# zengxianyu/sketchedit

Measured on NVIDIA H100. Metric: images/sec 256x256 CelebA-HQ generator fwd, higher is better.
Workload: dtype bf16

## Files before the change

sketchedit_b200/csrc/se_conv_c8.cu:

```cuda
#include "se_conv_c8.h"

#include <stdlib.h>

#include <atomic>
#include <map>
#include <mutex>
#include <vector>

#include "../../include/sketchedit_b200.h"
#include "se_tc_device.cuh"

namespace se {

constexpr int C8_TH = 16, C8_TW = 8;
constexpr int C8_CONSUMER_WARPS = 8;
__host__ __device__ constexpr int c8_threads(int teams) { return 32 * C8_CONSUMER_WARPS * teams + 32; }
constexpr int C8_MAX_STAGES = 8;

__device__ __forceinline__ void ring_of(int i, int n, int shift, int& slot, uint32_t& phase) {
  if (shift >= 0) { slot = i & (n - 1); phase = (uint32_t)(i >> shift) & 1u; }
  else { const int qd = i / n; slot = i - qd * n; phase = (uint32_t)qd & 1u; }
}

template <int NT, bool kF16, int R64, int M64, int R32, int TEAMS>
// ... 608 lines not shown
  }
  p.step_x = grid % p.tiles_x;
  p.step_y = (grid / p.tiles_x) % p.tiles_y;
  p.step_img = grid / (p.tiles_x * p.tiles_y);
  p.cstep_x = (teams * grid) % p.tiles_x;
  p.cstep_y = (teams * grid / p.tiles_x) % p.tiles_y;
  p.cstep_img = teams * grid / (p.tiles_x * p.tiles_y);
  cudaLaunchConfig_t cfg;
  cudaLaunchAttribute attr;
  c8_launch_config(&cfg, &attr, grid, teams, smem_bytes, p.cluster, stream);
  SE_CUDA_OK(cudaLaunchKernelEx(&cfg, kernel, tmA, p));
  if (c8_log_on()) c8_log_append(p, c, (int)(inst - kC8Insts), teams, grid, total_tiles);
  return 0;
}

}

extern "C" {

int se_c8_log_enable(int on) {
  std::lock_guard<std::mutex> lk(se::g_c8_log_mu);
  se::g_c8_log = on != 0;
  se::g_c8_log_recs.clear();
  se::g_c8_log_label.clear();
  return 0;
}

int se_c8_log_count(void) {
  std::lock_guard<std::mutex> lk(se::g_c8_log_mu);
  return (int)se::g_c8_log_recs.size();
// ... 28 lines not shown
```

sketchedit_b200/csrc/se_conv_c8.h:

```cpp
#pragma once
#include "se_common.cuh"
#include "se_conv_tc.h"

namespace se {

enum { C8_HALO = 0, C8_PERTAP = 1 };
constexpr int C8_MAX_ABUFS = 8;
constexpr int C8_MAX_UNITS = 128;

struct C8Layer {
  TcWeights w;
  int mode = C8_HALO;
  bool resident = false;
  bool stem = false;
  int cb_in = 0;
  int mmas64 = 4;
  int HR = 0, WR = 0;
  int pad_y0 = 0, pad_x0 = 0;
  int a_bytes = 0, a_tx_bytes = 0;
  int8_t tap_cb[MAX_TAPS] = {0};
  int chunks_per_tap = 1;
};

constexpr int C8_MAX_CLS = 4;
// ... 25 lines not shown
  const float* bias;
  EpiParams e;
  int f16;
  int8_t tap_cb[MAX_TAPS];
  int cpt;
  int ncls, cls_bytes;
  int cls_ooy[C8_MAX_CLS], cls_oox[C8_MAX_CLS];
  int cluster;
};

int c8_configure(C8Layer* L, int ntaps, const int8_t* dy, const int8_t* dx, int Ci, int Cout, bool stem, const int8_t* tap_cb = nullptr);
int c8_launch(const ConvParams& c, const C8Layer& L, cudaStream_t stream, const C8Group* grp = nullptr);
int c8_instantiated(const C8Layer& L, bool f16, const std::string& name);
int c8_configure_group(C8Group* G, int ncls, int ntaps, const int8_t (*dy)[8], const int8_t (*dx)[8], const int* ooy, const int* oox, int Ci, int Cout);

bool c8_log_on();
void c8_log_label(const std::string& name);

}
```

sketchedit_b200/csrc/se_engine.cu:

```cuda
#include <stdlib.h>

#include <cuda_fp16.h>

#include <algorithm>
#include <atomic>
#include <cmath>
#include <cstring>
#include <functional>
#include <map>
#include <mutex>
#include <string>
#include <type_traits>
#include <vector>

#include "../../include/sketchedit_b200.h"
#include "se_common.cuh"
#include "se_conv_direct.h"
#include "se_conv_c8.h"
#include "se_cam.h"
#include "se_gemm_split.h"
#include "se_conv_tc.h"
#include "se_misc.h"
#include "se_detail.h"

// ... 552 lines not shown
  } else {
    elems = (size_t)c.B * v.ld * (layout == 2 ? (size_t)(v.H / 2) * (v.W / 2) : (size_t)v.H * v.W) * 8;
  }
  t.bytes = elems * (dtype == 0 ? 4 : 2);
  SE_CUDA_OK(cudaMalloc(&t.p, t.bytes));
  c.m->taps.push_back(t);
  SE_CUDA_OK(cudaMemcpyAsync(t.p, v.p, t.bytes, cudaMemcpyDeviceToDevice, c.stream));
  return 0;
}
#define TAP(...)                  \
  do {                            \
    int _rt = tap(c, __VA_ARGS__); \
    if (_rt) return _rt;          \
  } while (0)

static int run_layer(Ctx& c, Layer& L, const View& in, void* out, int ldo, int choff, int out_c8 = 0) {
  SE_REQUIRE(in.c8 == wants_c8(c, L), "activation layout mismatch at layer " + L.name);
  TAP("in:" + std::string(1, L.net) + "." + L.name, in, L.is_stem ? 3 : in.c8);
  const Spec& s = L.spec;
  const int Ho = s.deconv ? in.H : (in.H + s.stride - 1) / s.stride;
  const int Wo = s.deconv ? in.W : (in.W + s.stride - 1) / s.stride;
  const bool fused = c.prec == SE_PREC_BF16_TC && !L.groups.empty() && in.c8 == 1;
  const bool split = c.split();
  const int n_launch = fused ? (int)L.groups.size() : (int)L.cls.size();
  if (c8_log_on() && !c.dry) c8_log_label(std::string(1, L.net) + "." + L.name);
  for (int li = 0; li < n_launch; ++li) {
    const C8Group* grp = fused ? &L.groups[li] : nullptr;
    ClassW& cw = L.cls[fused ? li * grp->ncls : li];
    ConvParams cp;
    memset(&cp, 0, sizeof(cp));
    cp.x = in.p; cp.in_dt = c.act_dt();
    cp.N = c.B; cp.Hi = in.H; cp.Wi = in.W; cp.Ci = L.Ci; cp.ldx = in.ld;
    if (L.is_stem && !in.c8) {
      cp.ldx = 8;
      cp.Wi = stem_wp(in.W) - 7;
      cp.x_row_pitch = (long long)stem_wp(in.W) * 8;
      cp.x_img_pitch = (long long)in.H * cp.x_row_pitch;
    }
    if (in.c8) {
      cp.in_c8 = 1; cp.x_cb_off = in.cb_off; cp.ldx = in.ld;
// ... 23 lines not shown
    cp.epi = s.act == 1 ? EPI_GATE_RELU : EPI_GATE_ELU;
    cp.scale = split ? 1.0f / (kSplitActScale * cw.s_wscale) : 1.0f;
    cp.colscale = nullptr;
    if (L.fused_pair) {
      SE_REQUIRE(out_c8 == 2 && ldo == 24, "a fused stem pair writes two space-to-depth tensors");
      cp.out_blk_split = 3; cp.out_par_stride = 3; cp.out_blk_jump = 9 * (cp.Hout / 2) * (cp.Wout / 2);
    }
    if (g_timing && !c.dry) {
      const double gc = grp ? grp->ncls : 1.0;
      const double pos = (double)c.B * Ho * Wo * gc, ncls = (double)L.cls.size() / gc;
      const double cin_alg = L.fused_pair ? L.pair_cin_sum / 2.0 : (double)s.cin;
      const double f_alg = 2.0 * pos * s.cout * cin_alg * (s.deconv ? 9.0 : (double)s.k * s.k);
      const double f_exec = 2.0 * pos * s.cout * cin_alg * (s.deconv ? 4.0 : (double)s.k * s.k) * (split ? 3.0 : 1.0);
      const double bytes = ((double)c.B * in.H * in.W * (L.fused_pair ? 8.0 : (double)s.cin) / ncls + pos * (s.cout / 2) + (double)s.cout * s.cin * s.k * s.k / ncls) * c.esz();
      char buf[160];
      snprintf(buf, sizeof(buf), "%s|%s %d->%d k%d s%d d%d @%dx%d", c.tc() ? (split ? "conv_c8_kernel (split-half fp16 x3)" : "conv_c8_kernel") : "conv_direct_kernel",
               s.deconv ? (grp ? (grp->ncls == 4 ? "deconv (4 classes fused)" : "deconv (2 classes fused)") : "deconv-class") : (L.fused_pair ? "stem pair" : "conv"), s.cin, s.cout, s.k, s.stride, s.rate, Ho * cw.osy, Wo * cw.osx);
      c.tag(buf, c.tc() ? 1 : 0, f_alg, f_exec, bytes);
    }
    if (split) CK(c8_launch(cp, cw.c8s, c.stream));
    else if (c.tc()) CK(c8_launch(cp, cw.c8, c.stream, grp));
    else {
      cp.w = cw.w_direct;
      CK(direct_launch(cp, cw.CoutP, c.stream));
    }
  }
  return 0;
}

static void out_dims(const Spec& s, int H, int W, int* Ho, int* Wo) {
  if (s.deconv) { *Ho = 2 * H; *Wo = 2 * W; }
  else { *Ho = (H + s.stride - 1) / s.stride; *Wo = (W + s.stride - 1) / s.stride; }
}

struct Dst { void* p = nullptr; int ld = 0, choff = 0, c8 = -1; };
// ... 32 lines not shown
  return 0;
}

static std::vector<std::string> with_prefix(const std::string& pfx, std::initializer_list<const char*> l, int skip = 0) {
  std::vector<std::string> v;
  for (auto s = l.begin() + skip; s != l.end(); ++s) v.push_back(pfx + *s);
  return v;
}

static int run_head(Ctx& c, char net, const std::string& name, const View& in, int mode, HeadIO io) {
  Layer* L = find_ready(c.m, net, name);
  SE_REQUIRE(L != nullptr && L->is_head, "head layer " + name + ": " + last_error());
  TAP("in:" + std::string(1, net) + "." + name, in, in.c8);
  {
    const double px = (double)c.B * in.H * in.W;
    const int outs = !!io.mask + !!io.mask_bin + !!io.stage + !!io.composed;
    const double bytes = px * ((in.c8 ? 16 : 12) * c.esz() + (io.img ? 12 : 0) + (io.blend ? 4 : 0) + outs * 4 * L->spec.cout + (io.packed ? 8 * c.esz() : 0));
    const double fl = 2.0 * px * 9 * 12 * L->spec.cout;
    c.tag(std::string("head_kernel|12->") + std::to_string(L->spec.cout) + " k3 + " +
              (mode == HEAD_MASK ? "sigmoid+threshold" : mode == HEAD_TANH ? "tanh" : mode == HEAD_COARSE ? "tanh+blend+pack8" : "tanh+soft blend"),
          0, fl, fl, bytes);
  }
  SE_REQUIRE(in.c8 == (c.tc() ? 1 : 0) && in.ld == (c.tc() ? 2 * c.sp() : 12), "head input: dense 12 channels in the mode's storage");
  io.x = in.p; io.B = c.B; io.H = in.H; io.W = in.W; io.mode = mode;
  io.Wp = stem_wp(in.W); io.padl = STEM_PADL; io.no_mask_coarse = c.m->opt[SE_OPT_NO_MASK_COARSE];
  CK(head(io, c.act_dt(), L->w_head_host.data(), L->b_host.data(), L->spec.cout, c.stream));
  return 0;
}

static int run_cam_tc(Ctx& c, const View& f, const float* mask_s, void* out, float* attn_out) {
  SE_REQUIRE(f.c8 == 2 && f.C == 96, "tensor-core attention reads a 96-channel space-to-depth channel-blocked map");
  CamPlan pl;
  int rc = cam_plan(c.B, f.H, f.W, c.attn_limit, attn_out != nullptr, &pl);
  if (rc) return rc;
  Buf fn = c.get(pl.fn_bytes), cs = c.get(pl.cs_bytes), P = c.get(pl.p_bytes);
  if (g_timing && !c.dry) {
    const double L = (double)pl.hs * pl.ws;
    const double fl = 4.0 * c.B * L * L * 96 * 16;
    c.tag("cam_s_kernel + cam_pv_kernel (+ norm, colscale)|contextual attention", 1, fl, 1.5 * fl,
          (double)c.B * f.H * f.W * 96 * 2 * 2 + 2.0 * (double)c.B * pl.KB * pl.hs * pl.ws * 16);
  }
// ... 152 lines not shown
  float* mask_bin = nullptr;
  unsigned char* mask_u8 = nullptr;
  float* x_stage1 = nullptr;
};

static int run_netM(Ctx& c, int H, int W, const NetMIO& io) {
  SE_REQUIRE(io.mask || io.x_stage1, "netM with neither output");
  Act in8, x9;
  int rc = do_pack8(c, &in8, io.x, io.guide, nullptr, H, W, PACK_IMG_ONE, 1.0f, 0);
  if (rc) return rc;
  std::vector<std::string> trunk = with_prefix("", kEncoder);
  trunk.pop_back();
  rc = run_chain(c, 'M', trunk, in8, &x9);
  if (rc) return rc;
  if (io.x_stage1) {
    Act v16;
    rc = run_chain(c, 'M', with_prefix("conv", kDecoder), x9.borrow(), &v16);
    if (rc) return rc;
    HeadIO h{};
    h.stage = io.x_stage1;
    rc = run_head(c, 'M', "conv17", v16.v, HEAD_TANH, h);
    if (rc) return rc;
    c.put(v16);
  }
  if (!io.mask) {
    c.put(x9);
    return 0;
  }
  Act v;
  rc = run_chain(c, 'M', with_prefix("", {"conv10_atrous", "conv_mask_11", "conv_mask_12", "conv_mask_13_upsample_conv", "conv_mask_14",
                                          "conv_mask_15_upsample_conv", "conv_mask_16"}),
                 x9, &v);
  if (rc) return rc;
  Buf scratch;
  HeadIO h{};
  h.mask = io.mask; h.mask_bs = io.mask_bs; h.mask_bin = io.mask_bin; h.mask_u8 = io.mask_u8;
  if (!h.mask_bin) { scratch = c.get((size_t)c.B * H * W * 4); h.mask_bin = (float*)scratch.p; }
  rc = run_head(c, 'M', "conv_mask_17", v.v, HEAD_MASK, h);
  if (rc) return rc;
  c.put(scratch);
  c.put(v);
  return 0;
}

static int run_stem_pair(Ctx& c, Layer& pair, Act in, Buf* st) {
  *st = c.get((size_t)c.B * 24 * (in.v.H / 2) * (in.v.W / 2) * 16);
  int rc = run_layer(c, pair, in.v, st->p, 24, 0, 2);
  if (rc) return rc;
  c.put(in);
  return 0;
}

struct NetGIO {
  const float *x, *x2, *mask, *mask2, *guide;
  float *x_stage1 = nullptr, *x_stage2 = nullptr, *composed = nullptr;
  long long composed_bs = 0;
// ... 27 lines not shown
  Act in;
  if (!pair1) rc = do_pack8(c, &in, io.x, io.guide, io.mask, H, W, PACK_IMG_ONE_MINUS_M, 1.0f, 1);
  if (rc) return rc;
  rc = run_chain(c, 'G', with_prefix("", kEncoder, pair1 ? 1 : 0), pair1 ? Act{pair_half(st1, 0)} : in, nullptr, Dst{cat1.p, cat_ld, 0});
  if (rc) return rc;
  if (!pair1) rc = do_pack8(c, &in, io.x2, io.guide, io.mask2, H, W, style_img, opt[SE_OPT_JOINT_TRAIN_INP] ? 0.0f : 1.0f, 1);
  if (rc) return rc;
  Act style;
  rc = run_chain(c, 'G', with_prefix("w", kEncoder, pair1 ? 1 : 0), pair1 ? Act{pair_half(st1, 1)} : in, &style);
  if (rc) return rc;
  c.put(st1);
  rc = do_pool_broadcast(c, style.v, opt[SE_OPT_POOL_AVG] ? RED_AVG : RED_MAX, cat1.p, cat_ld);
  if (rc) return rc;
  c.put(style);
  Buf xnow = c.get((size_t)c.B * H * stem_wp(W) * 8 * e);
  Act dec;
  rc = run_chain(c, 'G', with_prefix("conv", kDecoder), Act{c.dense(cat1.p, h, w, 192, tc), cat1}, &dec);
  if (rc) return rc;
  c.tag("memset|pad pixels of the packed stage-2 input", 0, 0, 0, (double)xnow.bytes);
  CK(fill_zero(xnow.p, xnow.bytes, c.stream));
  HeadIO coarse{};
  coarse.img = io.x; coarse.blend = io.mask; coarse.stage = io.x_stage1; coarse.packed = xnow.p;
  rc = run_head(c, 'G', "conv17", dec.v, HEAD_COARSE, coarse);
  if (rc) return rc;
  c.put(dec);

  Buf cat2 = c.get((size_t)c.B * h * w * 192 * e);
  Act in2{stem_view(c, xnow.p, H, W), xnow};
  Buf st2;
  if (pair2) {
    rc = run_stem_pair(c, *pair2, in2, &st2);
    if (rc) return rc;
  }
  rc = run_chain(c, 'G', with_prefix("x", kEncoder, pair2 ? 1 : 0), pair2 ? Act{pair_half(st2, 0)} : in2.borrow(), nullptr, Dst{cat2.p, cat_ld, 0});
  if (rc) return rc;
  const int pm_c8 = opt[SE_OPT_USE_CAM] ? (c.split() ? 1 : (tc ? 2 : 0)) : -1;
  Act pm;
  rc = run_chain(c, 'G', with_prefix("pm", {"conv1", "conv2_downsample", "conv3", "conv4_downsample", "conv5", "conv6"}, pair2 ? 1 : 0),
                 pair2 ? Act{pair_half(st2, 1), st2} : in2, &pm, Dst{nullptr, 0, 0, pm_c8});
  if (rc) return rc;
// ... 12 lines not shown
      rc = run_cam_split(c, (const float*)f32.p, h, w, 96, (const float*)ms.p, (float*)o32.p, io.attn);
      if (rc) return rc;
      TAP("out:G.cam.f32", nhwc(o32.p, h, w, 96, 96), 0, 0);
      CK(f32_to_act((const float*)o32.p, 1, camo.p, DT_F16X2, pml, c.B, 96, c.stream));
      c.put(o32); c.put(f32);
    } else {
      rc = tc ? run_cam_tc(c, pm.v, (const float*)ms.p, camo.p, io.attn) : run_cam(c, pm.v, (const float*)ms.p, camo.p, 96, io.attn, 0);
      if (rc) return rc;
    }
    c.put(ms);
    c.put(pm);
    pm = Act{c.dense(camo.p, h, w, 96, tc), camo};
  }
  rc = run_chain(c, 'G', with_prefix("pm", {"conv9", "conv10"}), pm, nullptr, Dst{cat2.p, cat_ld, 96});
  if (rc) return rc;
  rc = run_chain(c, 'G', with_prefix("allconv", kDecoder), Act{c.dense(cat2.p, h, w, 192, tc), cat2}, &dec);
  if (rc) return rc;
  HeadIO fine{};
  fine.stage = io.x_stage2;
  const bool blend = io.composed || io.composed_u8;
  if (blend) {
    fine.img = io.x; fine.blend = io.mask_soft; fine.blend_bs = io.msoft_bs;
    fine.composed = io.composed; fine.composed_bs = io.composed_bs; fine.bgr_u8 = io.composed_u8;
  }
  rc = run_head(c, 'G', "allconv17", dec.v, blend ? HEAD_FINE : HEAD_TANH, fine);
  if (rc) return rc;
  c.put(dec);
  return 0;
}

struct Request {
  const float *image = nullptr, *sketch = nullptr;
  const unsigned char *image_u8 = nullptr, *sketch_u8 = nullptr;
  const float* edit_mask = nullptr;
  const unsigned char* edit_mask_u8 = nullptr;
  float *composed = nullptr, *mask = nullptr;
  long long composed_bs = 0, mask_bs = 0;
  unsigned char *bgr_u8 = nullptr, *mask_u8 = nullptr;
  float *coarse = nullptr, *fine = nullptr, *mask_image = nullptr;
  const float* mask_bin_in = nullptr;
  float* mask_bin_out = nullptr;
  float* attn = nullptr;
// ... 610 lines not shown
```

sketchedit_b200/csrc/se_misc.cu:

```cuda
#include <type_traits>

#include "se_common.cuh"
#include "se_misc.h"

namespace se {

static inline int cdiv(long long a, long long b) { return (int)((a + b - 1) / b); }

struct F32 {
  static constexpr int kHalves = 1;
  static constexpr bool kBlocked = false;
  template <int N = 8>
  __device__ static void load8(const void* x, size_t o, size_t, float (&v)[8]) {
#pragma unroll
    for (int k = 0; k < N; ++k) v[k] = __ldg(static_cast<const float*>(x) + o + k);
  }
  __device__ static void store8(void* y, size_t o, size_t, const float (&v)[8]) {
#pragma unroll
    for (int k = 0; k < 8; ++k) static_cast<float*>(y)[o + k] = v[k];
  }
  __device__ static float get(const void* x, size_t o, size_t) { return __ldg(static_cast<const float*>(x) + o); }
  __device__ static void put(void* y, size_t o, size_t, float v) { static_cast<float*>(y)[o] = v; }
};

// ... 107 lines not shown
      for (int c = 0; c < 3; ++c) v[5 + c] = img[(b * 3 + c) * HW + pix] * a2;
    }
  }
  St::store8(out, o, lo, v);
}

int pack8(const float* img, const float* sketch, const float* mask, void* out, int dt, int B, int H, int W, int Wp, int padl,
          int img_mode, float sketch_scale, int write_mask, cudaStream_t s, int img2_mode) {
  const long long n = (long long)B * H * Wp;
  return with_storage(dt, [&](auto st) {
    pack8_kernel<decltype(st)><<<cdiv(n, 256), 256, 0, s>>>(img, sketch, mask, out, B, H, W, Wp, padl, img_mode, sketch_scale, write_mask,
                                                            img2_mode);
  });
}

template <int COUT>
struct HeadWeights {
  float2 w[9][6][COUT];
  float b[COUT];
};
template <class St, int COUT>
__global__ void __launch_bounds__(128) head_kernel(const __grid_constant__ HeadWeights<COUT> hw, const __grid_constant__ HeadIO io) {
  constexpr bool kPairs = std::is_same<St, Bf16>::value;
  const int H = io.H, W = io.W;
  const long long i = blockIdx.x * (long long)blockDim.x + threadIdx.x;
  const long long HW = (long long)H * W;
  if (i >= io.B * HW) return;
  const long long b = i / HW, pix = i % HW;
  const int yy = (int)(pix / W), xx = (int)(pix % W);
  float2 acc[COUT];
#pragma unroll
  for (int o = 0; o < COUT; ++o) acc[o] = make_float2(kPairs ? 0.0f : hw.b[o], 0.0f);
#pragma unroll
  for (int t = 0; t < 9; ++t) {
    const int iy = yy + t / 3 - 1, ix = xx + t % 3 - 1;
    if (iy < 0 || iy >= H || ix < 0 || ix >= W) continue;
    const long long q = (long long)iy * W + ix;
    float v[2][8];
    if constexpr (St::kBlocked) {
      const size_t o = ((size_t)b * 2 * St::kHalves * HW + q) * 8, blk = (size_t)HW * 8;
      St::load8(io.x, o, 2 * blk, v[0]);
      St::load8(io.x, o + blk, 2 * blk, v[1]);
    } else {
      St::load8(io.x, (size_t)(b * HW + q) * 12, 0, v[0]);
      St::template load8<4>(io.x, (size_t)(b * HW + q) * 12 + 8, 0, v[1]);
    }
#pragma unroll
    for (int p = 0; p < 6; ++p) {
      const float xe = v[p / 4][(2 * p) % 8], xo = v[p / 4][(2 * p + 1) % 8];
#pragma unroll
      for (int o = 0; o < COUT; ++o) {
        const float2 wv = hw.w[t][p][o];
        if (kPairs) {
          acc[o].x = fmaf(xe, wv.x, acc[o].x);
          acc[o].y = fmaf(xo, wv.y, acc[o].y);
        } else {
          acc[o].x = fmaf(xo, wv.y, fmaf(xe, wv.x, acc[o].x));
        }
      }
    }
  }
  float r[COUT];
#pragma unroll
  for (int o = 0; o < COUT; ++o) r[o] = kPairs ? hw.b[o] + (acc[o].x + acc[o].y) : acc[o].x;
  if (io.mode == HEAD_MASK) {
    const float sg = 1.0f / (1.0f + expf(-r[0]));
    io.mask[b * io.mask_bs + pix] = sg;
    io.mask_bin[i] = sg > 0.5f ? 1.0f : 0.0f;
    if (io.mask_u8) io.mask_u8[i] = (unsigned char)(int)(sg * 255.0f);
    return;
  }
  float t3[COUT];
#pragma unroll
  for (int o = 0; o < COUT; ++o) t3[o] = tanhf(r[o]);
  if (io.mode == HEAD_TANH) {
#pragma unroll
    for (int o = 0; o < COUT; ++o) io.stage[(b * COUT + o) * HW + pix] = t3[o];
  } else if (io.mode == HEAD_COARSE) {
    const float m = io.blend[i];
    float pk[8];
#pragma unroll
    for (int o = 0; o < 8; ++o) pk[o] = 0.0f;
#pragma unroll
    for (int o = 0; o < COUT; ++o) {
      if (io.stage) io.stage[(b * COUT + o) * HW + pix] = t3[o];
      const float xin = io.img[(b * 3 + o) * HW + pix] * (1.0f - m);
      pk[o] = io.no_mask_coarse ? t3[o] : (t3[o] * m + xin * (1.0f - m));
    }
    const size_t o = (((size_t)b * St::kHalves * H + yy) * io.Wp + xx + io.padl) * 8;
    St::store8(io.packed, o, (size_t)H * io.Wp * 8, pk);
  } else {
    const float m = io.blend[b * io.blend_bs + pix];
#pragma unroll
    for (int o = 0; o < COUT; ++o) {
      if (io.stage) io.stage[(b * COUT + o) * HW + pix] = t3[o];
      const float cv = t3[o] * m + io.img[(b * 3 + o) * HW + pix] * (1.0f - m);
      if (io.composed) io.composed[b * io.composed_bs + o * HW + pix] = cv;
      if (io.bgr_u8) io.bgr_u8[i * 3 + (2 - o)] = (unsigned char)(int)((cv + 1.0f) / 2.0f * 255.0f);
    }
  }
}

template <int COUT>
static int head_launch(HeadIO io, int dt, const float* w_host, const float* b_host, cudaStream_t s) {
  HeadWeights<COUT> hw;
  for (int t = 0; t < 9; ++t)
    for (int p = 0; p < 6; ++p)
      for (int o = 0; o < COUT; ++o) hw.w[t][p][o] = make_float2(w_host[(t * 12 + 2 * p) * COUT + o], w_host[(t * 12 + 2 * p + 1) * COUT + o]);
  for (int o = 0; o < COUT; ++o) hw.b[o] = b_host[o];
  const long long HW = (long long)io.H * io.W;
  if (!io.blend_bs) io.blend_bs = HW;
  if (!io.mask_bs) io.mask_bs = HW;
  if (!io.composed_bs) io.composed_bs = 3 * HW;
  return with_storage(dt, [&](auto st) { head_kernel<decltype(st), COUT><<<cdiv(io.B * HW, 128), 128, 0, s>>>(hw, io); });
}
int head(HeadIO io, int dt, const float* w_host, const float* b_host, int cout, cudaStream_t s) {
  SE_REQUIRE(cout == 1 || cout == 3, "head cout");
  return cout == 1 ? head_launch<1>(io, dt, w_host, b_host, s) : head_launch<3>(io, dt, w_host, b_host, s);
}

__global__ void plane_reduce_kernel(const float* __restrict__ x, int ldx, int C, int HW, int mode, float* __restrict__ out) {
  __shared__ float red[8][33];
  const int b = blockIdx.y;
  const int c = blockIdx.x * 32 + threadIdx.x;
  float acc = (mode == RED_MAX) ? -INFINITY : 0.0f;
  if (c < C) {
    const float* xp = x + (size_t)b * HW * ldx + c;
#pragma unroll 4
// ... 339 lines not shown
```

Baseline: 5211.

## Fuse last 24->24 decoder conv with 3x3 output head via shared-memory row ring

Adds a persistent kernel that runs the final 24-channel 3x3 gated conv with WGMMA over vertical strips of the image. The gated result goes into a small shared-memory ring of row tiles, and the 12->COUT head conv plus its tanh, blend or mask epilogue is computed from that ring two tile-rows behind. This removes a kernel launch and the global write and re-read of the intermediate activation. The head logic is moved into a shared header so both paths use it. In exchange the kernel carries a 2-row-tile pipeline lag with extra barriers, and it only applies when N*strips fills the SMs.

```diff
diff --git a/sketchedit_b200/csrc/se_conv_c8.cu b/sketchedit_b200/csrc/se_conv_c8.cu
--- a/sketchedit_b200/csrc/se_conv_c8.cu
+++ b/sketchedit_b200/csrc/se_conv_c8.cu
@@ -8,6 +8,7 @@
 #include <vector>
 
 #include "../../include/sketchedit_b200.h"
+#include "se_head.cuh"
 #include "se_tc_device.cuh"
 
 namespace se {
@@ -646,6 +647,261 @@
   return 0;
 }
 
+
+struct C8HeadParams {
+  int N, H, W, strips, tiles_y;
+  int a_bytes, a_tx_bytes, x_cb_off, wres_bytes;
+  int lbo_bytes, sbo_bytes, kstep_bytes;
+  uint32_t aoff[9];
+  const uint8_t* w;
+  const float* bias;
+  EpiParams e;
+};
+constexpr int C8H_COLS = 14, C8H_ABUFS = 2, C8H_SLOTS = 4;
+constexpr int C8H_SLOT_ELEMS = 2 * C8_TH * 16 * 8;
+
+template <int COUT>
+__global__ void __launch_bounds__(c8_threads(1), 2)
+conv_c8_head_kernel(const __grid_constant__ CUtensorMap tmA, const __grid_constant__ C8HeadParams p,
+                    const __grid_constant__ HeadWeights<COUT> hw, const __grid_constant__ HeadIO io) {
+  constexpr int NT = 32;
+  extern __shared__ __align__(1024) uint8_t smem_raw[];
+  uint8_t* smem = reinterpret_cast<uint8_t*>((reinterpret_cast<uintptr_t>(smem_raw) + 1023) & ~uintptr_t(1023));
+  uint8_t* sHalo = smem;
+  uint8_t* sWres = sHalo + C8H_ABUFS * p.a_bytes;
+  __nv_bfloat16* ring = reinterpret_cast<__nv_bfloat16*>(sWres + p.wres_bytes);
+  uint64_t* a_full = reinterpret_cast<uint64_t*>(ring + C8H_SLOTS * C8H_SLOT_ELEMS);
+  uint64_t* a_empty = a_full + C8H_ABUFS;
+  uint64_t* wres_bar = a_empty + C8H_ABUFS;
+  float* bias_s = reinterpret_cast<float*>(wres_bar + 2);
+  const int warp = threadIdx.x >> 5, lane = threadIdx.x & 31;
+  if (threadIdx.x == 0) {
+    for (int i = 0; i < C8H_ABUFS; ++i) {
+      mbar_init(&a_full[i], 1);
+      mbar_init(&a_empty[i], C8_CONSUMER_WARPS);
+    }
+    mbar_init(wres_bar, 1);
+    asm volatile("fence.mbarrier_init.release.cluster;" ::: "memory");
+  }
+  epi_fill_constants(bias_s, NT + 32, p.bias, p.e, threadIdx.x, c8_threads(1));
+  __syncthreads();
+  const int items = p.N * p.strips, T = p.tiles_y;
+
+  if (warp == C8_CONSUMER_WARPS) {
+    if (elect_one()) {
+      asm volatile("prefetch.tensormap [%0];" ::"l"(reinterpret_cast<uint64_t>(&tmA)) : "memory");
+      mbar_expect_tx(wres_bar, (uint32_t)p.wres_bytes);
+      bulk_load_1d(sWres, p.w, (uint32_t)p.wres_bytes, wres_bar);
+    }
+    __syncwarp();
+    int iter = 0;
+    for (int item = blockIdx.x; item < items; item += gridDim.x) {
+      const int img = item / p.strips, x0 = C8H_COLS * (item - img * p.strips) - 1;
+      for (int ty = 0; ty < T; ++ty, ++iter) {
+        const int ab = iter & 1;
+        mbar_wait(&a_empty[ab], ((iter >> 1) & 1) ^ 1, 5);
+        if (elect_one()) {
+          mbar_expect_tx(&a_full[ab], (uint32_t)p.a_tx_bytes);
+          tma_load_4d(sHalo + (size_t)ab * p.a_bytes, &tmA, &a_full[ab], (x0 - 1) * 8, ty * C8_TH - 1, p.x_cb_off, img);
+        }
+        __syncwarp();
+      }
+    }
+  } else {
+    const int tid = threadIdx.x, wg = warp >> 2, wq = warp & 3;
+    const uint32_t smem_base = smem_u32(smem);
+    const uint32_t sB = smem_base + (uint32_t)(C8H_ABUFS * p.a_bytes);
+    const uint32_t cst_s = smem_u32(bias_s);
+    const bool elu = p.e.epi == EPI_GATE_ELU;
+    EpiParams er = p.e;
+    er.y = ring;
+    er.blk_stride = C8_TH * 16 * 8;
+    er.blk_split = 1 << 20;
+    er.blk_jump = 0;
+    const bool ok[2] = {true, true};
+    const int hr = tid / C8H_COLS, hc = tid - hr * C8H_COLS;
+    const long long HW = (long long)p.H * p.W;
+    mbar_wait(wres_bar, 0, 6);
+    float acc[2][NT / 2];
+#pragma unroll
+    for (int c = 0; c < 2; ++c)
+#pragma unroll
+      for (int i = 0; i < NT / 2; ++i) acc[c][i] = 0.0f;
+    int iter = 0;
+    for (int item = blockIdx.x; item < items; item += gridDim.x) {
+      const int img = item / p.strips, s = item - img * p.strips;
+      for (int ty = 0; ty < T + 2; ++ty) {
+        const bool conv = ty < T;
+        const int ab = iter & 1;
+        const int hy = ty - 2, y = hy * C8_TH + hr, x = C8H_COLS * s + hc;
+        const long long pix = (long long)min(max(y, 0), p.H - 1) * p.W + min(x, p.W - 1), i = img * HW + pix;
+        const HeadIn<COUT> hin = head_inputs<COUT>(io, img, pix, i, HW);
+        if (conv) {
+          mbar_wait(&a_full[ab], (iter >> 1) & 1, 7);
+          const uint32_t sA = smem_base + (uint32_t)(ab * p.a_bytes) + (uint32_t)wg * 8u * (uint32_t)p.sbo_bytes;
+          wg_fence();
+          wg_fence_acc(acc[0]);
+          wg_fence_acc(acc[1]);
+#pragma unroll
+          for (int c = 0; c < 2; ++c)
+#pragma unroll
+            for (int j = 0; j < 9; ++j) {
+              const uint32_t a0 = sA + p.aoff[j] + (uint32_t)c * 8u * 16u;
+              const uint32_t b0 = sB + (uint32_t)(j * NT * 64);
+#pragma unroll
+              for (int k = 0; k < 2; ++k)
+                Wgmma<NT, false, 0>::mma(acc[c], wg_desc(a0 + k * p.kstep_bytes, p.lbo_bytes, p.sbo_bytes, WG_SW_NONE),
+                                         wg_desc(b0 + 32u * k, 16u, 512u, WG_SW64), j + k ? 1u : 0u);
+            }
+          wg_commit();
+        }
+        if (conv) {
+          wg_wait<0>();
+          wg_fence_acc(acc[0]);
+          wg_fence_acc(acc[1]);
+          __syncwarp();
+          if (lane == 0) mbar_arrive(&a_empty[ab]);
+          ++iter;
+#pragma unroll
+          for (int c = 0; c < 2; ++c) {
+            size_t base[2];
+#pragma unroll
+            for (int h = 0; h < 2; ++h)
+              base[h] = (size_t)(ty & (C8H_SLOTS - 1)) * C8H_SLOT_ELEMS + (size_t)(((8 * wg + 2 * wq + h) * 16 + 8 * c + (lane >> 2)) * 8 + 2 * (lane & 3));
+            if (elu) conv_epilogue<NT, false, true, true>(er, cst_s, acc[c], base, ok, lane);
+            else conv_epilogue<NT, false, false, true>(er, cst_s, acc[c], base, ok, lane);
+          }
+        }
+        if (ty >= 2 && tid < C8_TH * C8H_COLS) {
+          if (y < p.H && x < p.W) {
+            float2 hacc[COUT];
+#pragma unroll
+            for (int o = 0; o < COUT; ++o) hacc[o] = make_float2(0.0f, 0.0f);
+#pragma unroll
+            for (int t = 0; t < 9; ++t) {
+              const int iy = y + t / 3 - 1, ix = x + t % 3 - 1;
+              if (iy < 0 || iy >= p.H || ix < 0 || ix >= p.W) continue;
+              const __nv_bfloat16* q = ring + ((iy >> 4) & (C8H_SLOTS - 1)) * C8H_SLOT_ELEMS + ((iy & 15) * 16 + hc + t % 3) * 8;
+              float v[2][8];
+#pragma unroll
+              for (int blk = 0; blk < 2; ++blk) {
+                const uint4 w4 = *reinterpret_cast<const uint4*>(q + blk * (C8_TH * 16 * 8));
+                const uint32_t wd[4] = {w4.x, w4.y, w4.z, w4.w};
+#pragma unroll
+                for (int k = 0; k < 4; ++k) {
+                  v[blk][2 * k] = __uint_as_float(wd[k] << 16);
+                  v[blk][2 * k + 1] = __uint_as_float(wd[k] & 0xffff0000u);
+                }
+              }
+              head_tap<COUT, true>(hw, t, v, hacc);
+            }
+            float r[COUT];
+#pragma unroll
+            for (int o = 0; o < COUT; ++o) r[o] = hw.b[o] + (hacc[o].x + hacc[o].y);
+            float pk[8];
+            if (head_outputs<COUT>(io, r, hin, img, pix, i, HW, pk)) {
+              const size_t o = (((size_t)img * p.H + y) * io.Wp + x + io.padl) * 8;
+              *reinterpret_cast<uint4*>(static_cast<__nv_bfloat16*>(io.packed) + o) =
+                  make_uint4(pack_bf16x2(pk[0], pk[1]), pack_bf16x2(pk[2], pk[3]), pack_bf16x2(pk[4], pk[5]), pack_bf16x2(pk[6], pk[7]));
+            }
+          }
+        }
+        named_bar_sync(1, 32 * C8_CONSUMER_WARPS);
+      }
+    }
+  }
+}
+
+template <int COUT>
+static int c8_head_set_smem(int bytes) {
+  static std::atomic<int> done{0};
+  if (done.load() < bytes) {
+    SE_CUDA_OK(cudaFuncSetAttribute(conv_c8_head_kernel<COUT>, cudaFuncAttributeMaxDynamicSharedMemorySize, bytes));
+    done.store(bytes);
+  }
+  return 0;
+}
+
+bool c8_head_fills(int N, int W) {
+  int dev = 0, sms = 0;
+  if (cudaGetDevice(&dev) != cudaSuccess || cudaDeviceGetAttribute(&sms, cudaDevAttrMultiProcessorCount, dev) != cudaSuccess) return false;
+  return (long long)N * ((W + C8H_COLS - 1) / C8H_COLS) >= sms;
+}
+
+int c8_head_launch(const ConvParams& c, const C8Layer& L, HeadIO io, const float* w_head, const float* b_head, int cout, cudaStream_t stream) {
+  const TcWeights& w = L.w;
+  SE_REQUIRE(cout == 1 || cout == 3, "head cout");
+  SE_REQUIRE(c.in_dt == DT_BF16 && c.out_dt == DT_BF16 && !c.f16x2 && c.in_c8 == 1, "the fused conv16 + head runs the bf16 path");
+  SE_REQUIRE(c.stride == 1 && c.ntaps == 9 && w.ntaps == 9 && w.NT == 32 && w.n64 == 0 && w.n32 == 1 && L.resident && L.mode == C8_HALO &&
+                 L.cb_in == 4 && c.Cout == 24,
+             "the fused conv16 + head is a 24 -> 24 3x3 layer with resident weights");
+  SE_REQUIRE(c.epi == EPI_GATE_ELU || c.epi == EPI_GATE_RELU, "conv_c8 runs gated epilogues only");
+  SE_REQUIRE((reinterpret_cast<uintptr_t>(c.x) & 127) == 0, "input base must be 128 B aligned");
+  SE_REQUIRE(c.Ho == c.Hi && c.Wo == c.Wi && c.Hout == c.Ho && c.Wout == c.Wo && c.osy == 1 && c.osx == 1, "a stride-1 layer");
+  C8HeadParams p;
+  memset(&p, 0, sizeof(p));
+  p.N = c.N; p.H = c.Ho; p.W = c.Wo;
+  p.strips = (c.Wo + C8H_COLS - 1) / C8H_COLS;
+  p.tiles_y = (c.Ho + C8_TH - 1) / C8_TH;
+  const int HR = C8_TH + 2, WR = 2 * C8_TW + 2;
+  p.a_tx_bytes = L.cb_in * HR * WR * 16;
+  p.a_bytes = (p.a_tx_bytes + 1023) / 1024 * 1024;
+  p.x_cb_off = c.x_cb_off;
+  p.wres_bytes = (int)tc_weight_bytes_per_image(w);
+  p.lbo_bytes = HR * WR * 16; p.kstep_bytes = 2 * p.lbo_bytes; p.sbo_bytes = WR * 16;
+  for (int t = 0; t < 9; ++t) {
+    SE_REQUIRE(c.dy[t] >= -1 && c.dy[t] <= 1 && c.dx[t] >= -1 && c.dx[t] <= 1 && c.tap_cb[t] == 0, "3x3 taps of dilation 1");
+    p.aoff[t] = (uint32_t)(((c.dy[t] + 1) * WR + (c.dx[t] + 1)) * 16);
+  }
+  p.w = reinterpret_cast<const uint8_t*>(w.data);
+  p.bias = c.bias;
+  fill_epi(c, w.NT, &p.e);
+  SE_REQUIRE(p.e.paired, "the ring stores channel pairs");
+  io.B = c.N; io.H = c.Ho; io.W = c.Wo;
+  head_io_strides(&io);
+  const int smem_bytes = 1024 + C8H_ABUFS * p.a_bytes + p.wres_bytes + C8H_SLOTS * C8H_SLOT_ELEMS * 2 + (2 * C8H_ABUFS + 2) * 8 + 3 * (32 + 32) * 4 + 64;
+  EncodeTiledFn enc = c8_encode_fn();
+  SE_REQUIRE(enc != nullptr, "cuTensorMapEncodeTiled not available from the driver");
+  int dev = 0, sms = 0;
+  SE_CUDA_OK(cudaGetDevice(&dev));
+  SE_CUDA_OK(cudaDeviceGetAttribute(&sms, cudaDevAttrMultiProcessorCount, dev));
+  CUtensorMap tmA;
+  {
+    cuuint64_t dims[4] = {(cuuint64_t)c.Wi * 8, (cuuint64_t)c.Hi, (cuuint64_t)c.ldx, (cuuint64_t)c.N};
+    cuuint64_t strides[3] = {(cuuint64_t)c.Wi * 16, (cuuint64_t)c.Hi * c.Wi * 16, (cuuint64_t)c.ldx * c.Hi * c.Wi * 16};
+    cuuint32_t box[4] = {(cuuint32_t)(WR * 8), (cuuint32_t)HR, (cuuint32_t)L.cb_in, 1};
+    cuuint32_t estr[4] = {1, 1, 1, 1};
+    CUresult r = enc(&tmA, CU_TENSOR_MAP_DATA_TYPE_BFLOAT16, 4, const_cast<void*>(c.x), dims, strides, box, estr,
+                     CU_TENSOR_MAP_INTERLEAVE_NONE, CU_TENSOR_MAP_SWIZZLE_NONE, CU_TENSOR_MAP_L2_PROMOTION_L2_256B,
+                     CU_TENSOR_MAP_FLOAT_OOB_FILL_NONE);
+    SE_REQUIRE(r == CUDA_SUCCESS, "cuTensorMapEncodeTiled(C8 strips) failed, CUresult=" + std::to_string((int)r));
+  }
+  const int items = p.N * p.strips;
+  const int grid = items < 2 * sms ? items : 2 * sms;
+  if (cout == 1) {
+    { int rc = c8_head_set_smem<1>(smem_bytes); if (rc) return rc; }
+    conv_c8_head_kernel<1><<<grid, c8_threads(1), smem_bytes, stream>>>(tmA, p, head_weights<1>(w_head, b_head), io);
+  } else {
+    { int rc = c8_head_set_smem<3>(smem_bytes); if (rc) return rc; }
+    conv_c8_head_kernel<3><<<grid, c8_threads(1), smem_bytes, stream>>>(tmA, p, head_weights<3>(w_head, b_head), io);
+  }
+  SE_CUDA_OK(cudaGetLastError());
+  if (c8_log_on()) {
+    C8LogEntry e;
+    memset(e.rec, 0, sizeof(e.rec));
+    int* r = e.rec;
+    r[SE_C8_INST] = -1; r[SE_C8_TEAMS] = 1; r[SE_C8_CLUSTER] = 1; r[SE_C8_GRID] = grid;
+    r[SE_C8_TOTAL_TILES] = items; r[SE_C8_N] = p.N; r[SE_C8_TILES_X] = p.strips; r[SE_C8_TILES_Y] = p.tiles_y;
+    r[SE_C8_HO] = p.H; r[SE_C8_WO] = p.W;
+    r[SE_C8_MODE] = C8_HEAD_STRIPS; r[SE_C8_CPT] = 1; r[SE_C8_NCLS] = 1; r[SE_C8_A_BUFS] = C8H_ABUFS;
+    r[SE_C8_NUM_STAGES] = cout;
+    std::lock_guard<std::mutex> lk(g_c8_log_mu);
+    e.name = g_c8_log_label;
+    g_c8_log_recs.push_back(e);
+  }
+  return 0;
+}
+
 }
 
 extern "C" {
diff --git a/sketchedit_b200/csrc/se_conv_c8.h b/sketchedit_b200/csrc/se_conv_c8.h
--- a/sketchedit_b200/csrc/se_conv_c8.h
+++ b/sketchedit_b200/csrc/se_conv_c8.h
@@ -1,10 +1,11 @@
 #pragma once
 #include "se_common.cuh"
 #include "se_conv_tc.h"
+#include "se_misc.h"
 
 namespace se {
 
-enum { C8_HALO = 0, C8_PERTAP = 1 };
+enum { C8_HALO = 0, C8_PERTAP = 1, C8_HEAD_STRIPS = 2 };
 constexpr int C8_MAX_ABUFS = 8;
 constexpr int C8_MAX_UNITS = 128;
 
@@ -63,6 +64,9 @@
 int c8_instantiated(const C8Layer& L, bool f16, const std::string& name);
 int c8_configure_group(C8Group* G, int ncls, int ntaps, const int8_t (*dy)[8], const int8_t (*dx)[8], const int* ooy, const int* oox, int Ci, int Cout);
 
+bool c8_head_fills(int N, int W);
+int c8_head_launch(const ConvParams& c, const C8Layer& L, HeadIO io, const float* w_head, const float* b_head, int cout, cudaStream_t stream);
+
 bool c8_log_on();
 void c8_log_label(const std::string& name);
 
diff --git a/sketchedit_b200/csrc/se_engine.cu b/sketchedit_b200/csrc/se_engine.cu
--- a/sketchedit_b200/csrc/se_engine.cu
+++ b/sketchedit_b200/csrc/se_engine.cu
@@ -590,7 +590,16 @@
     if (_rt) return _rt;          \
   } while (0)
 
-static int run_layer(Ctx& c, Layer& L, const View& in, void* out, int ldo, int choff, int out_c8 = 0) {
+struct HeadFuse { const Layer* L; int mode; HeadIO io; };
+static const char* head_mode_name(int mode) {
+  return mode == HEAD_MASK ? "sigmoid+threshold" : mode == HEAD_TANH ? "tanh" : mode == HEAD_COARSE ? "tanh+blend+pack8" : "tanh+soft blend";
+}
+static double head_side_bytes(const Ctx& c, const HeadIO& io, int cout) {
+  const int outs = !!io.mask + !!io.mask_bin + !!io.stage + !!io.composed;
+  return (io.img ? 12 : 0) + (io.blend ? 4 : 0) + outs * 4 * cout + (io.packed ? 8 * c.esz() : 0);
+}
+
+static int run_layer(Ctx& c, Layer& L, const View& in, void* out, int ldo, int choff, int out_c8 = 0, const HeadFuse* hf = nullptr) {
   SE_REQUIRE(in.c8 == wants_c8(c, L), "activation layout mismatch at layer " + L.name);
   TAP("in:" + std::string(1, L.net) + "." + L.name, in, L.is_stem ? 3 : in.c8);
   const Spec& s = L.spec;
@@ -599,7 +608,7 @@
   const bool fused = c.prec == SE_PREC_BF16_TC && !L.groups.empty() && in.c8 == 1;
   const bool split = c.split();
   const int n_launch = fused ? (int)L.groups.size() : (int)L.cls.size();
-  if (c8_log_on() && !c.dry) c8_log_label(std::string(1, L.net) + "." + L.name);
+  if (c8_log_on() && !c.dry) c8_log_label(std::string(1, L.net) + "." + L.name + (hf ? "+" + hf->L->name : ""));
   for (int li = 0; li < n_launch; ++li) {
     const C8Group* grp = fused ? &L.groups[li] : nullptr;
     ClassW& cw = L.cls[fused ? li * grp->ncls : li];
@@ -653,11 +662,21 @@
       const double f_exec = 2.0 * pos * s.cout * cin_alg * (s.deconv ? 4.0 : (double)s.k * s.k) * (split ? 3.0 : 1.0);
       const double bytes = ((double)c.B * in.H * in.W * (L.fused_pair ? 8.0 : (double)s.cin) / ncls + pos * (s.cout / 2) + (double)s.cout * s.cin * s.k * s.k / ncls) * c.esz();
       char buf[160];
+      if (hf) {
+        const int hc = hf->L->spec.cout;
+        const double fh = 2.0 * pos * 9 * 12 * hc;
+        snprintf(buf, sizeof(buf), "conv_c8_head_kernel|conv %d->%d k3 + head 12->%d k3 + %s @%dx%d", s.cin, s.cout, hc, head_mode_name(hf->mode), Ho, Wo);
+        c.tag(buf, 1, f_alg + fh, f_exec + fh, bytes - pos * (s.cout / 2) * c.esz() + pos * head_side_bytes(c, hf->io, hc));
+      } else {
       snprintf(buf, sizeof(buf), "%s|%s %d->%d k%d s%d d%d @%dx%d", c.tc() ? (split ? "conv_c8_kernel (split-half fp16 x3)" : "conv_c8_kernel") : "conv_direct_kernel",
                s.deconv ? (grp ? (grp->ncls == 4 ? "deconv (4 classes fused)" : "deconv (2 classes fused)") : "deconv-class") : (L.fused_pair ? "stem pair" : "conv"), s.cin, s.cout, s.k, s.stride, s.rate, Ho * cw.osy, Wo * cw.osx);
       c.tag(buf, c.tc() ? 1 : 0, f_alg, f_exec, bytes);
-    }
-    if (split) CK(c8_launch(cp, cw.c8s, c.stream));
+      }
+    }
+    if (hf) {
+      SE_REQUIRE(c.prec == SE_PREC_BF16_TC && !grp && n_launch == 1, "a fused head follows a plain bf16 tensor-core layer");
+      CK(c8_head_launch(cp, cw.c8, hf->io, hf->L->w_head_host.data(), hf->L->b_host.data(), hf->L->spec.cout, c.stream));
+    } else if (split) CK(c8_launch(cp, cw.c8s, c.stream));
     else if (c.tc()) CK(c8_launch(cp, cw.c8, c.stream, grp));
     else {
       cp.w = cw.w_direct;
@@ -720,17 +739,41 @@
   TAP("in:" + std::string(1, net) + "." + name, in, in.c8);
   {
     const double px = (double)c.B * in.H * in.W;
-    const int outs = !!io.mask + !!io.mask_bin + !!io.stage + !!io.composed;
-    const double bytes = px * ((in.c8 ? 16 : 12) * c.esz() + (io.img ? 12 : 0) + (io.blend ? 4 : 0) + outs * 4 * L->spec.cout + (io.packed ? 8 * c.esz() : 0));
+    const double bytes = px * ((in.c8 ? 16 : 12) * c.esz() + head_side_bytes(c, io, L->spec.cout));
     const double fl = 2.0 * px * 9 * 12 * L->spec.cout;
-    c.tag(std::string("head_kernel|12->") + std::to_string(L->spec.cout) + " k3 + " +
-              (mode == HEAD_MASK ? "sigmoid+threshold" : mode == HEAD_TANH ? "tanh" : mode == HEAD_COARSE ? "tanh+blend+pack8" : "tanh+soft blend"),
-          0, fl, fl, bytes);
+    c.tag(std::string("head_kernel|12->") + std::to_string(L->spec.cout) + " k3 + " + head_mode_name(mode), 0, fl, fl, bytes);
   }
   SE_REQUIRE(in.c8 == (c.tc() ? 1 : 0) && in.ld == (c.tc() ? 2 * c.sp() : 12), "head input: dense 12 channels in the mode's storage");
   io.x = in.p; io.B = c.B; io.H = in.H; io.W = in.W; io.mode = mode;
   io.Wp = stem_wp(in.W); io.padl = STEM_PADL; io.no_mask_coarse = c.m->opt[SE_OPT_NO_MASK_COARSE];
   CK(head(io, c.act_dt(), L->w_head_host.data(), L->b_host.data(), L->spec.cout, c.stream));
+  return 0;
+}
+
+static int run_decoder_tail(Ctx& c, char net, std::vector<std::string> chain, Act in, const std::string& head, int mode, HeadIO io) {
+  Act x;
+  if (c.prec != SE_PREC_BF16_TC || c.m->taps_on || !c8_head_fills(c.B, in.v.W * 4)) {
+    int rc = run_chain(c, net, chain, in, &x);
+    if (rc) return rc;
+    rc = run_head(c, net, head, x.v, mode, io);
+    if (rc) return rc;
+    c.put(x);
+    return 0;
+  }
+  const std::string l16 = chain.back();
+  chain.pop_back();
+  int rc = run_chain(c, net, chain, in, &x);
+  if (rc) return rc;
+  Layer* L = find_ready(c.m, net, l16);
+  SE_REQUIRE(L != nullptr, "unknown or unloaded layer " + l16 + ": " + last_error());
+  const Layer* LH = find_ready(c.m, net, head);
+  SE_REQUIRE(LH != nullptr && LH->is_head, "head layer " + head + ": " + last_error());
+  io.mode = mode;
+  io.Wp = stem_wp(x.v.W); io.padl = STEM_PADL; io.no_mask_coarse = c.m->opt[SE_OPT_NO_MASK_COARSE];
+  const HeadFuse hf{LH, mode, io};
+  rc = run_layer(c, *L, x.v, nullptr, 0, 0, 1, &hf);
+  if (rc) return rc;
+  c.put(x);
   return 0;
 }
 
@@ -913,32 +956,24 @@
   rc = run_chain(c, 'M', trunk, in8, &x9);
   if (rc) return rc;
   if (io.x_stage1) {
-    Act v16;
-    rc = run_chain(c, 'M', with_prefix("conv", kDecoder), x9.borrow(), &v16);
-    if (rc) return rc;
     HeadIO h{};
     h.stage = io.x_stage1;
-    rc = run_head(c, 'M', "conv17", v16.v, HEAD_TANH, h);
+    rc = run_decoder_tail(c, 'M', with_prefix("conv", kDecoder), x9.borrow(), "conv17", HEAD_TANH, h);
     if (rc) return rc;
-    c.put(v16);
   }
   if (!io.mask) {
     c.put(x9);
     return 0;
   }
-  Act v;
-  rc = run_chain(c, 'M', with_prefix("", {"conv10_atrous", "conv_mask_11", "conv_mask_12", "conv_mask_13_upsample_conv", "conv_mask_14",
-                                          "conv_mask_15_upsample_conv", "conv_mask_16"}),
-                 x9, &v);
-  if (rc) return rc;
   Buf scratch;
   HeadIO h{};
   h.mask = io.mask; h.mask_bs = io.mask_bs; h.mask_bin = io.mask_bin; h.mask_u8 = io.mask_u8;
   if (!h.mask_bin) { scratch = c.get((size_t)c.B * H * W * 4); h.mask_bin = (float*)scratch.p; }
-  rc = run_head(c, 'M', "conv_mask_17", v.v, HEAD_MASK, h);
+  rc = run_decoder_tail(c, 'M', with_prefix("", {"conv10_atrous", "conv_mask_11", "conv_mask_12", "conv_mask_13_upsample_conv", "conv_mask_14",
+                                                 "conv_mask_15_upsample_conv", "conv_mask_16"}),
+                        x9, "conv_mask_17", HEAD_MASK, h);
   if (rc) return rc;
   c.put(scratch);
-  c.put(v);
   return 0;
 }
 
@@ -996,16 +1031,12 @@
   if (rc) return rc;
   c.put(style);
   Buf xnow = c.get((size_t)c.B * H * stem_wp(W) * 8 * e);
-  Act dec;
-  rc = run_chain(c, 'G', with_prefix("conv", kDecoder), Act{c.dense(cat1.p, h, w, 192, tc), cat1}, &dec);
-  if (rc) return rc;
   c.tag("memset|pad pixels of the packed stage-2 input", 0, 0, 0, (double)xnow.bytes);
   CK(fill_zero(xnow.p, xnow.bytes, c.stream));
   HeadIO coarse{};
   coarse.img = io.x; coarse.blend = io.mask; coarse.stage = io.x_stage1; coarse.packed = xnow.p;
-  rc = run_head(c, 'G', "conv17", dec.v, HEAD_COARSE, coarse);
-  if (rc) return rc;
-  c.put(dec);
+  rc = run_decoder_tail(c, 'G', with_prefix("conv", kDecoder), Act{c.dense(cat1.p, h, w, 192, tc), cat1}, "conv17", HEAD_COARSE, coarse);
+  if (rc) return rc;
 
   Buf cat2 = c.get((size_t)c.B * h * w * 192 * e);
   Act in2{stem_view(c, xnow.p, H, W), xnow};
@@ -1048,8 +1079,6 @@
   }
   rc = run_chain(c, 'G', with_prefix("pm", {"conv9", "conv10"}), pm, nullptr, Dst{cat2.p, cat_ld, 96});
   if (rc) return rc;
-  rc = run_chain(c, 'G', with_prefix("allconv", kDecoder), Act{c.dense(cat2.p, h, w, 192, tc), cat2}, &dec);
-  if (rc) return rc;
   HeadIO fine{};
   fine.stage = io.x_stage2;
   const bool blend = io.composed || io.composed_u8;
@@ -1057,9 +1086,8 @@
     fine.img = io.x; fine.blend = io.mask_soft; fine.blend_bs = io.msoft_bs;
     fine.composed = io.composed; fine.composed_bs = io.composed_bs; fine.bgr_u8 = io.composed_u8;
   }
-  rc = run_head(c, 'G', "allconv17", dec.v, blend ? HEAD_FINE : HEAD_TANH, fine);
-  if (rc) return rc;
-  c.put(dec);
+  rc = run_decoder_tail(c, 'G', with_prefix("allconv", kDecoder), Act{c.dense(cat2.p, h, w, 192, tc), cat2}, "allconv17", blend ? HEAD_FINE : HEAD_TANH, fine);
+  if (rc) return rc;
   return 0;
 }
 
diff --git a/sketchedit_b200/csrc/se_head.cuh b/sketchedit_b200/csrc/se_head.cuh
--- /dev/null
+++ b/sketchedit_b200/csrc/se_head.cuh
@@ -0,0 +1,103 @@
+#pragma once
+#include "se_common.cuh"
+#include "se_misc.h"
+
+namespace se {
+
+template <int COUT>
+struct HeadWeights {
+  float2 w[9][6][COUT];
+  float b[COUT];
+};
+template <int COUT>
+HeadWeights<COUT> head_weights(const float* w_host, const float* b_host) {
+  HeadWeights<COUT> hw;
+  for (int t = 0; t < 9; ++t)
+    for (int p = 0; p < 6; ++p)
+      for (int o = 0; o < COUT; ++o) hw.w[t][p][o] = make_float2(w_host[(t * 12 + 2 * p) * COUT + o], w_host[(t * 12 + 2 * p + 1) * COUT + o]);
+  for (int o = 0; o < COUT; ++o) hw.b[o] = b_host[o];
+  return hw;
+}
+inline void head_io_strides(HeadIO* io) {
+  const long long HW = (long long)io->H * io->W;
+  if (!io->blend_bs) io->blend_bs = HW;
+  if (!io->mask_bs) io->mask_bs = HW;
+  if (!io->composed_bs) io->composed_bs = 3 * HW;
+}
+
+template <int COUT, bool kPairs>
+__device__ __forceinline__ void head_tap(const HeadWeights<COUT>& hw, int t, const float (&v)[2][8], float2 (&acc)[COUT]) {
+#pragma unroll
+  for (int p = 0; p < 6; ++p) {
+    const float xe = v[p / 4][(2 * p) % 8], xo = v[p / 4][(2 * p + 1) % 8];
+#pragma unroll
+    for (int o = 0; o < COUT; ++o) {
+      const float2 wv = hw.w[t][p][o];
+      if (kPairs) {
+        acc[o].x = fmaf(xe, wv.x, acc[o].x);
+        acc[o].y = fmaf(xo, wv.y, acc[o].y);
+      } else {
+        acc[o].x = fmaf(xo, wv.y, fmaf(xe, wv.x, acc[o].x));
+      }
+    }
+  }
+}
+
+template <int COUT>
+struct HeadIn { float m, img[COUT]; };
+template <int COUT>
+__device__ __forceinline__ HeadIn<COUT> head_inputs(const HeadIO& io, long long b, long long pix, long long i, long long HW) {
+  HeadIn<COUT> in;
+  in.m = 0.0f;
+#pragma unroll
+  for (int o = 0; o < COUT; ++o) in.img[o] = 0.0f;
+  if (io.mode == HEAD_COARSE || io.mode == HEAD_FINE) {
+    in.m = io.blend[io.mode == HEAD_COARSE ? i : b * io.blend_bs + pix];
+#pragma unroll
+    for (int o = 0; o < COUT; ++o) in.img[o] = io.img[(b * 3 + o) * HW + pix];
+  }
+  return in;
+}
+
+template <int COUT>
+__device__ __forceinline__ bool head_outputs(const HeadIO& io, const float (&r)[COUT], const HeadIn<COUT>& in, long long b, long long pix,
+                                             long long i, long long HW, float (&pk)[8]) {
+  if (io.mode == HEAD_MASK) {
+    const float sg = 1.0f / (1.0f + expf(-r[0]));
+    io.mask[b * io.mask_bs + pix] = sg;
+    io.mask_bin[i] = sg > 0.5f ? 1.0f : 0.0f;
+    if (io.mask_u8) io.mask_u8[i] = (unsigned char)(int)(sg * 255.0f);
+    return false;
+  }
+  float t3[COUT];
+#pragma unroll
+  for (int o = 0; o < COUT; ++o) t3[o] = tanhf(r[o]);
+  if (io.mode == HEAD_TANH) {
+#pragma unroll
+    for (int o = 0; o < COUT; ++o) io.stage[(b * COUT + o) * HW + pix] = t3[o];
+    return false;
+  }
+  if (io.mode == HEAD_COARSE) {
+    const float m = in.m, om = 1.0f - m;
+#pragma unroll
+    for (int o = 0; o < 8; ++o) pk[o] = 0.0f;
+#pragma unroll
+    for (int o = 0; o < COUT; ++o) {
+      if (io.stage) io.stage[(b * COUT + o) * HW + pix] = t3[o];
+      const float xin = in.img[o] * om;
+      pk[o] = io.no_mask_coarse ? t3[o] : fmaf(om, xin, t3[o] * m);
+    }
+    return true;
+  }
+  const float m = in.m;
+#pragma unroll
+  for (int o = 0; o < COUT; ++o) {
+    if (io.stage) io.stage[(b * COUT + o) * HW + pix] = t3[o];
+    const float cv = fmaf(t3[o], m, in.img[o] * (1.0f - m));
+    if (io.composed) io.composed[b * io.composed_bs + o * HW + pix] = cv;
+    if (io.bgr_u8) io.bgr_u8[i * 3 + (2 - o)] = (unsigned char)(int)((cv + 1.0f) / 2.0f * 255.0f);
+  }
+  return false;
+}
+
+}
diff --git a/sketchedit_b200/csrc/se_misc.cu b/sketchedit_b200/csrc/se_misc.cu
--- a/sketchedit_b200/csrc/se_misc.cu
+++ b/sketchedit_b200/csrc/se_misc.cu
@@ -1,6 +1,7 @@
 #include <type_traits>
 
 #include "se_common.cuh"
+#include "se_head.cuh"
 #include "se_misc.h"
 
 namespace se {
@@ -145,11 +146,6 @@
   });
 }
 
-template <int COUT>
-struct HeadWeights {
-  float2 w[9][6][COUT];
-  float b[COUT];
-};
 template <class St, int COUT>
 __global__ void __launch_bounds__(128) head_kernel(const __grid_constant__ HeadWeights<COUT> hw, const __grid_constant__ HeadIO io) {
   constexpr bool kPairs = std::is_same<St, Bf16>::value;
@@ -176,73 +172,23 @@
       St::load8(io.x, (size_t)(b * HW + q) * 12, 0, v[0]);
       St::template load8<4>(io.x, (size_t)(b * HW + q) * 12 + 8, 0, v[1]);
     }
-#pragma unroll
-    for (int p = 0; p < 6; ++p) {
-      const float xe = v[p / 4][(2 * p) % 8], xo = v[p / 4][(2 * p + 1) % 8];
-#pragma unroll
-      for (int o = 0; o < COUT; ++o) {
-        const float2 wv = hw.w[t][p][o];
-        if (kPairs) {
-          acc[o].x = fmaf(xe, wv.x, acc[o].x);
-          acc[o].y = fmaf(xo, wv.y, acc[o].y);
-        } else {
-          acc[o].x = fmaf(xo, wv.y, fmaf(xe, wv.x, acc[o].x));
-        }
-      }
-    }
+    head_tap<COUT, kPairs>(hw, t, v, acc);
   }
   float r[COUT];
 #pragma unroll
   for (int o = 0; o < COUT; ++o) r[o] = kPairs ? hw.b[o] + (acc[o].x + acc[o].y) : acc[o].x;
-  if (io.mode == HEAD_MASK) {
-    const float sg = 1.0f / (1.0f + expf(-r[0]));
-    io.mask[b * io.mask_bs + pix] = sg;
-    io.mask_bin[i] = sg > 0.5f ? 1.0f : 0.0f;
-    if (io.mask_u8) io.mask_u8[i] = (unsigned char)(int)(sg * 255.0f);
-    return;
-  }
-  float t3[COUT];
-#pragma unroll
-  for (int o = 0; o < COUT; ++o) t3[o] = tanhf(r[o]);
-  if (io.mode == HEAD_TANH) {
-#pragma unroll
-    for (int o = 0; o < COUT; ++o) io.stage[(b * COUT + o) * HW + pix] = t3[o];
-  } else if (io.mode == HEAD_COARSE) {
-    const float m = io.blend[i];
-    float pk[8];
-#pragma unroll
-    for (int o = 0; o < 8; ++o) pk[o] = 0.0f;
-#pragma unroll
-    for (int o = 0; o < COUT; ++o) {
-      if (io.stage) io.stage[(b * COUT + o) * HW + pix] = t3[o];
-      const float xin = io.img[(b * 3 + o) * HW + pix] * (1.0f - m);
-      pk[o] = io.no_mask_coarse ? t3[o] : (t3[o] * m + xin * (1.0f - m));
-    }
+  float pk[8];
+  if (head_outputs<COUT>(io, r, head_inputs<COUT>(io, b, pix, i, HW), b, pix, i, HW, pk)) {
     const size_t o = (((size_t)b * St::kHalves * H + yy) * io.Wp + xx + io.padl) * 8;
     St::store8(io.packed, o, (size_t)H * io.Wp * 8, pk);
-  } else {
-    const float m = io.blend[b * io.blend_bs + pix];
-#pragma unroll
-    for (int o = 0; o < COUT; ++o) {
-      if (io.stage) io.stage[(b * COUT + o) * HW + pix] = t3[o];
-      const float cv = t3[o] * m + io.img[(b * 3 + o) * HW + pix] * (1.0f - m);
-      if (io.composed) io.composed[b * io.composed_bs + o * HW + pix] = cv;
-      if (io.bgr_u8) io.bgr_u8[i * 3 + (2 - o)] = (unsigned char)(int)((cv + 1.0f) / 2.0f * 255.0f);
-    }
   }
 }
 
 template <int COUT>
 static int head_launch(HeadIO io, int dt, const float* w_host, const float* b_host, cudaStream_t s) {
-  HeadWeights<COUT> hw;
-  for (int t = 0; t < 9; ++t)
-    for (int p = 0; p < 6; ++p)
-      for (int o = 0; o < COUT; ++o) hw.w[t][p][o] = make_float2(w_host[(t * 12 + 2 * p) * COUT + o], w_host[(t * 12 + 2 * p + 1) * COUT + o]);
-  for (int o = 0; o < COUT; ++o) hw.b[o] = b_host[o];
+  const HeadWeights<COUT> hw = head_weights<COUT>(w_host, b_host);
+  head_io_strides(&io);
   const long long HW = (long long)io.H * io.W;
-  if (!io.blend_bs) io.blend_bs = HW;
-  if (!io.mask_bs) io.mask_bs = HW;
-  if (!io.composed_bs) io.composed_bs = 3 * HW;
   return with_storage(dt, [&](auto st) { head_kernel<decltype(st), COUT><<<cdiv(io.B * HW, 128), 128, 0, s>>>(hw, io); });
 }
 int head(HeadIO io, int dt, const float* w_host, const float* b_host, int cout, cudaStream_t s) {
```

Result: faster. 5264, median of 6 (+1.0%).
